# ZeldaM1/PnP-VCVE

Hardware: AMD Instinct MI355X
Metric: enhanced frames/sec (1280x720, 7-frame window) (higher is better)
Workload: dtype f32; 1 GPU; 1 x 7x3x720x1280 clip per GPU per step (BASELINE configs[2] shape), full BAE+CAA forward, config HR_davis_LR_128x128 generator, seeded random weights; side info per SURVEY 8(d): partition class ~ U{0,1,2} per 8x8 block (one-hot/255, none on the I frame), quarter-pel block MVs, IBBBP cadence; vsr_x4_heads=False, hip_graphs=False, deform=vos, parallelism=clip-sharded replicas x1

## Files before the change

### include/pnpvcve.h

```cpp
#ifndef PNPVCVE_H
#define PNPVCVE_H
#include <stddef.h>
#include <stdint.h>
#ifdef __cplusplus
extern "C" {
#endif

#define PNP_ERR_BAD_ARG 1001
#define PNP_ERR_UNSUPPORTED 1002
#define PNP_ERR_WORKSPACE 1003
#define PNP_ERR_SIZE_ASSERT 1004
#define PNP_ERR_SIZE_VALUE 1005

int pnp_abi_version(void);

typedef struct pnp_generator_cfg {
    int mid_channels;
    int num_blocks;
    int num_experts;
    int with_cat, use_base_qp, expert_softmax, with_bias, with_se;
    int one_layer, channel_first, align_key, vsr;
    int deform;
    int sparse_val;
    int num_group;
// ... 31 lines not shown
#define PNP_OPT_TILE_QUEUE 8
#define PNP_OPT_WINOGRAD 9
#define PNP_WINO_UNITS_MAX_TILES 128
#define PNP_OPT_COUNT 10
int pnp_generator_set_option(pnp_generator* g, int option, int value);
int pnp_generator_get_option(const pnp_generator* g, int option);

int pnp_generator_pack(const pnp_generator* g, const float* flat_dev, float* packed_dev, void* stream);

#define PNP_MAX_CONTEXTS 8
int64_t pnp_generator_workspace_bytes(const pnp_generator* g, int t, int h, int w);

int pnp_generator_set_max_resident(pnp_generator* g, int k);
int pnp_generator_get_max_resident(const pnp_generator* g);
int pnp_generator_min_resident(const pnp_generator* g, int t);

int pnp_generator_forward(const pnp_generator* g, const float* flat_dev, const float* packed_dev,
                          const float* lrs_dev, const float* mvs_dev, const float* par_dev,
                          const float* slices_host, const float* qps_host, const float* base_qps_host,
                          float* out_dev, void* workspace_dev, int64_t workspace_bytes,
                          int n, int t, int h, int w, void* stream);

#define PNP_PROF_CONV_BLOCK 0
#define PNP_PROF_CONV_INPUT 1
#define PNP_PROF_CONV_HEAD 2
#define PNP_PROF_WARP 3
#define PNP_PROF_DCN 4
int pnp_generator_profile(pnp_generator* g, int enable);
int pnp_generator_profile_read(pnp_generator* g, int kind, double* total_ms, int64_t* launches, double* work);

// ... 93 lines not shown
```

### include/pnpvcve_debug.h

```cpp
#ifndef PNPVCVE_DEBUG_H
#define PNPVCVE_DEBUG_H
#include "pnpvcve.h"
#ifdef __cplusplus
extern "C" {
#endif

#define PNP_CONV_AUTO 0
#define PNP_CONV_TILE 1
#define PNP_CONV_TILE_BIG 2

int pnp_conv3x3_f32_ex(int nsrc, const float* const* srcs_dev, const int* src_channels,
                       const float* const* packed_w_dev, const float* bias_dev, const float* gamma_dev,
                       const float* packed_w1x1_dev, const float* par_dev, const float* residual_dev,
                       int act, float* out_dev, int h, int w, int variant, const int* par_flags_dev,
                       void* trace_dev, void* stream);

int pnp_conv3x3_wino_f32_ex(const float* src_dev, const float* wino_w_dev, const float* bias_dev, const float* gamma_dev,
                            const float* wino_w1x1_dev, const float* par_dev, const int* par_flags_dev,
                            const float* residual_dev, int act, float* out_dev, int h, int w, void* trace_dev, void* stream);
int pnp_debug_wino_gate_word(const int* gate_word_dev);

int pnp_conv3x3_f16_ex(int nsrc, const float* const* srcs_dev, const int* src_channels,
                       const void* const* packed_w_f16_dev, const float* bias_dev, const float* gamma_dev,
                       const void* packed_w1x1_f16_dev, const float* par_dev, const float* residual_dev,
                       int act, float* out_dev, int h, int w, void* trace_dev, void* stream);

int pnp_dcn_trace_u64s(void);
int pnp_dcn_nhwc_f32_ex(const float* x_dev, const float* om_dev, const float* flow_x_dev, const float* flow_y_dev,
                        const float* w_packed_dev, const float* bias_dev, float* out_dev, int h, int w, void* trace_dev,
                        void* stream);

int pnp_conv3x3_f16_maps(int nsrc, const void* const* srcs_dev, const int* src_channels, int src_f16_mask,
                         const void* const* packed_w_f16_dev, const float* bias_dev, const float* gamma_dev,
                         const void* packed_w1x1_f16_dev, const float* par_dev, const int* par_flags_dev,
                         const float* residual_dev, int act, void* out_dev, int out_f16, void* out16_dev, int h, int w,
// ... 16 lines not shown
```

### pnp_vcve_amd/_native.py

```python
import ctypes
import os
from ctypes import POINTER, c_char_p, c_float, c_int, c_int64, c_void_p

_HERE = os.path.dirname(os.path.abspath(__file__))
LIB_PATH = os.path.join(_HERE, 'lib', 'libpnpvcve_hip.so')

PNP_ERR = {1001: 'bad argument', 1002: 'unsupported configuration', 1003: 'workspace too small or misaligned',
           1004: 'size assert', 1005: 'size value'}


class GeneratorCfg(ctypes.Structure):
    _fields_ = [(k, c_int) for k in (
        'mid_channels', 'num_blocks', 'num_experts', 'with_cat', 'use_base_qp', 'expert_softmax', 'with_bias',
        'with_se', 'one_layer', 'channel_first', 'align_key', 'vsr', 'deform', 'sparse_val', 'num_group', 'flow_inter',
        'blocktype')]


SIGNATURES = {
    'pnp_abi_version': (c_int, []),
    'pnp_generator_create': (c_int, [POINTER(GeneratorCfg), POINTER(c_void_p)]),
    'pnp_generator_destroy': (None, [c_void_p]),
    'pnp_generator_num_params': (c_int, [c_void_p]),
    'pnp_generator_param_name': (c_char_p, [c_void_p, c_int]),
    'pnp_generator_param_ndim': (c_int, [c_void_p, c_int]),
    'pnp_generator_param_dim': (c_int64, [c_void_p, c_int, c_int]),
    'pnp_generator_param_offset': (c_int64, [c_void_p, c_int]),
    'pnp_generator_flat_floats': (c_int64, [c_void_p]),
    'pnp_generator_packed_floats': (c_int64, [c_void_p]),
    'pnp_generator_pack': (c_int, [c_void_p, c_void_p, c_void_p, c_void_p]),
    'pnp_generator_workspace_bytes': (c_int64, [c_void_p, c_int, c_int, c_int]),
    'pnp_generator_set_max_resident': (c_int, [c_void_p, c_int]),
    'pnp_generator_get_max_resident': (c_int, [c_void_p]),
    'pnp_generator_min_resident': (c_int, [c_void_p, c_int]),
    'pnp_generator_forward': (c_int, [c_void_p, c_void_p, c_void_p, c_void_p, c_void_p, c_void_p,
                                      POINTER(c_float), POINTER(c_float), POINTER(c_float),
                                      c_void_p, c_void_p, c_int64, c_int, c_int, c_int, c_int, c_void_p]),
    'pnp_generator_set_precision': (c_int, [c_void_p, c_int]),
    'pnp_generator_get_precision': (c_int, [c_void_p]),
    'pnp_generator_set_option': (c_int, [c_void_p, c_int, c_int]),
    'pnp_generator_get_option': (c_int, [c_void_p, c_int]),
    'pnp_generator_profile': (c_int, [c_void_p, c_int]),
    'pnp_generator_profile_read': (c_int, [c_void_p, c_int, POINTER(ctypes.c_double), POINTER(c_int64),
                                           POINTER(ctypes.c_double)]),
    'pnp_flow_warp_nchw_f32': (c_int, [c_void_p, c_void_p, c_void_p, c_int, c_int, c_int, c_int, c_void_p]),
    'pnp_mv_warp_nhwc_f32': (c_int, [c_void_p, c_void_p, c_void_p, c_void_p, c_int, c_int, c_int, c_void_p]),
    'pnp_flow_warp_nchw_mode_f32': (c_int, [c_void_p, c_void_p, c_void_p, c_int, c_int, c_int, c_int, c_int, c_void_p]),
    'pnp_mv_warp_nhwc_mode_f32': (c_int, [c_void_p, c_void_p, c_void_p, c_void_p, c_int, c_int, c_int, c_int, c_void_p]),
# ... 46 lines not shown
    'pnp_conv3x3_f16x3_ex': (c_int, [c_int, POINTER(c_void_p), POINTER(c_int), POINTER(c_void_p), POINTER(c_void_p),
                                     c_void_p, c_void_p, c_void_p, c_void_p, c_void_p, c_void_p,
                                     c_int, c_void_p, c_int, c_int, c_int, c_void_p, c_void_p, c_void_p]),
    'pnp_conv3x3_f32_ex': (c_int, [c_int, POINTER(c_void_p), POINTER(c_int), POINTER(c_void_p), c_void_p, c_void_p,
                                   c_void_p, c_void_p, c_void_p, c_int, c_void_p, c_int, c_int, c_int, c_void_p,
                                   c_void_p, c_void_p]),
    'pnp_conv3x3_f16_ex': (c_int, [c_int, POINTER(c_void_p), POINTER(c_int), POINTER(c_void_p), c_void_p, c_void_p,
                                   c_void_p, c_void_p, c_void_p, c_int, c_void_p, c_int, c_int, c_void_p, c_void_p]),
}

DEBUG_SIGNATURES['pnp_dcn_nhwc_f32_ex'] = (c_int, [c_void_p, c_void_p, c_void_p, c_void_p, c_void_p, c_void_p, c_void_p, c_int,
                                                   c_int, c_void_p, c_void_p])

DEBUG_SIGNATURES['pnp_dcn_trace_u64s'] = (c_int, [])
DEBUG_SIGNATURES['pnp_debug_wino_gate_word'] = (c_int, [c_void_p])
DEBUG_SIGNATURES['pnp_conv3x3_wino_f32_ex'] = (c_int, [c_void_p] * 8 + [c_int, c_void_p, c_int, c_int, c_void_p, c_void_p])
DEBUG_SIGNATURES['pnp_conv3x3_f16_maps'] = (c_int, [c_int, POINTER(c_void_p), POINTER(c_int), c_int, POINTER(c_void_p), c_void_p,
                                                    c_void_p, c_void_p, c_void_p, c_void_p, c_void_p, c_int, c_void_p, c_int, c_void_p,
                                                    c_int, c_int, c_int, c_void_p, c_void_p])
DEBUG_SIGNATURES['pnp_mv_warp_nhwc_f16out'] = (c_int, [c_void_p, c_void_p, c_void_p, c_void_p, c_int, c_int, c_int, c_void_p])

(OPT_F16_MAPS, OPT_PAR_SKIP, OPT_CONV_LAST_VALU, OPT_PERSIST, OPT_SMALL_F16, OPT_SPARSE_EVAL, OPT_F16_MIRRORS, OPT_F16_CHAIN_MIRRORS,
 OPT_TILE_QUEUE, OPT_WINOGRAD) = range(10)
CONV_AUTO, CONV_TILE, CONV_TILE_BIG = range(3)
WINO_UNITS_MAX_TILES = 128


def wino_kernel_form(h, w, wopt):
    if wopt <= 0:
        return None
# ... 34 lines not shown
```

### pnp_vcve_amd/csrc/conv_mfma.h

```cpp
#pragma once
#include "common.h"

struct ConvArgs {
    const float* src[4];
    const float* wsrc[4];
    int src_c[4];
    int nsrc;
    const float* wpar;
    const float* wwino;
    const float* wwino_par;
    const float* wwino_src[4];
    const float* wwino_rgb;
    const int* par_any;
    int wino_units;
    const float* wvalu;
    const void* wsrc_h[4];
    const void* wpar_h;
    int wpar_h_scaled;
    int* tile_queue;
    int prec;
    int src_f16, out_f16;
    void* out16;
    int no_multi16;
    const float* par;
    const int* par_flags;
    long par_plane;
    const float* bias;
    const float* gamma;
// ... 93 lines not shown
```

### pnp_vcve_amd/csrc/conv_wino.hip

```cpp
#include "conv_mfma.h"
#include <cstring>
#include <type_traits>

namespace {

template <int N>
using I = std::integral_constant<int, N>;
typedef unsigned u32x4 __attribute__((ext_vector_type(4)));

constexpr int HP = 18, NPX = HP * HP;
constexpr int SLAB_B = NPX * 64;
constexpr int RING_B = 4 * 16384;
constexpr int PV_B = RING_B + 4 * SLAB_B;
constexpr int BG_B = PV_B + 256 * 48;
constexpr int DUMP_B = BG_B + 256;
constexpr int WINO_LDS = DUMP_B + 1024;
constexpr unsigned OOBW = 0xFFFFFFF0u;

__device__ __forceinline__ f32x4 mfma16(float a, float b, f32x4 c) { return __builtin_amdgcn_mfma_f32_16x16x4f32(a, b, c, 0, 0, 0); }
__device__ __forceinline__ __amdgpu_buffer_rsrc_t rsrc_of(const void* p, unsigned bytes) {
    return __builtin_amdgcn_make_buffer_rsrc(const_cast<void*>(p), 0, __builtin_amdgcn_readfirstlane((int)bytes), 0x00020000);
}
__device__ __forceinline__ f32x4 bload4(__amdgpu_buffer_rsrc_t r, unsigned voff, unsigned soff) {
    return __builtin_bit_cast(f32x4, __builtin_amdgcn_raw_buffer_load_b128(r, (int)voff, (int)soff, 0));
// ... 25 lines not shown
    long par_plane;
    const int* par_flags;
    const float *bias, *gamma, *residual;
    float* out;
    int H, W, act;
    unsigned long long* dbg;
    const float* srcs[3];
    unsigned u_off[3];
    const float* ubase;
    int nsrc;
    const float* rgb;
    const float* Urgb;
    const int* gate;
    int gate_mask, gate_want;
    int quad;
};

template <bool PAR, bool RES, bool MS, bool FO = false>
__device__ __forceinline__ void wino_tile_body(const WinoArgs& a) {
    static_assert(!MS || (!PAR && !RES), "the multi-source form is the input conv: no branches, no residual");
    static_assert(!FO || (!PAR && !MS), "fold-only is the plain structure");
    extern __shared__ __attribute__((aligned(16))) char smem[];
    const int t = threadIdx.x, lane = t & 63, wave = t >> 6;
    const int m = lane & 15, kq = lane >> 4;
    const int H = a.H, W = a.W;
    const int tiles_x = (W + 15) >> 4, ntiles = tiles_x * ((H + 15) >> 4);
    constexpr bool MSF = MS;
    constexpr bool SEAM = PAR;
    if (a.gate) {
        const int gv = __builtin_nontemporal_load(a.gate);
        if (((gv & a.gate_mask) != 0) != (a.gate_want != 0)) return;
    }

    int tile, tstep, tend, qtile = -1, qquad = 0;
    if ((gridDim.x & 7) == 0) {
        const int xcd = blockIdx.x & 7, slot = blockIdx.x >> 3;
        const int bq = ntiles >> 3, br = ntiles & 7;
        const int xbeg = xcd < br ? xcd * (bq + 1) : br * (bq + 1) + (xcd - br) * bq;
        tend = xbeg + bq + (xcd < br ? 1 : 0);
        tile = xbeg + slot;
        tstep = gridDim.x >> 3;
        const int nband = tend - xbeg, rounds = nband / tstep, left = nband - rounds * tstep;
        if (!MS && a.quad && rounds >= 1 && left > 0 && 4 * left <= tstep) {
            tend = xbeg + rounds * tstep;
            if (slot < 4 * left) {
                qtile = tend + (slot >> 2);
                qquad = slot & 3;
            }
        }
    } else {
        tile = blockIdx.x;
        tstep = gridDim.x;
        tend = ntiles;
    }
    if (tile >= tend) return;

    const unsigned map_bytes = (unsigned)H * (unsigned)W * 256u;
    __amdgpu_buffer_rsrc_t r_src = rsrc_of(reinterpret_cast<const char*>(MS ? a.srcs[0] : a.src) - ((long)W + 1) * 256, OOBW);
    const __amdgpu_buffer_rsrc_t r_u = rsrc_of(MS ? a.ubase : a.U, MS ? OOBW : 16u * 16384u);
    const __amdgpu_buffer_rsrc_t r_urgb = rsrc_of(MS ? a.Urgb : a.U, 4u * 4096u);
    const __amdgpu_buffer_rsrc_t r_rgb = rsrc_of(reinterpret_cast<const char*>(MS ? a.rgb : a.src) - ((long)W + 1) * 16, OOBW);
    const __amdgpu_buffer_rsrc_t r_up = rsrc_of((PAR || FO) ? a.Upar : a.U, 4u * 12288u);
    const __amdgpu_buffer_rsrc_t r_out = rsrc_of(a.out, map_bytes);
    const __amdgpu_buffer_rsrc_t r_res = rsrc_of(RES ? a.residual : a.src, RES ? map_bytes : 0u);
    const __amdgpu_buffer_rsrc_t r_par = rsrc_of(a.par, PAR ? (unsigned)(3 * a.par_plane * 4) : 0u);

    const unsigned t16 = (unsigned)t * 16u;
    const int ty = 4 * (wave >> 1) + (m >> 2), tx = 4 * (wave & 1) + (m & 3);
// ... 1279 lines not shown
    if (!a.wwino_rgb || a.prec != 0 || cfg == CONV_CFG_RGB || grid_y != 1 || a.out_mode != 0) return false;
    if (a.nsrc < 2 || a.nsrc > 4 || a.src_c[0] != 4 || a.src_f16 || a.out_f16 || a.out16) return false;
    if (a.wpar || a.residual || a.gamma) return false;
    for (int s = 1; s < a.nsrc; ++s)
        if (a.src_c[s] != 64 || !a.wwino_src[s]) return false;
    return (long)a.H * a.W * 256 < ((long)1 << 32) - 65536;
}

bool conv_wino_eligible(const ConvArgs& a, int cfg, int grid_y) {
    if (!a.wwino || a.prec != 0 || cfg == CONV_CFG_RGB || grid_y != 1 || a.out_mode != 0) return false;
    if (a.nsrc != 1 || a.src_c[0] != 64 || a.src_f16 || a.out_f16 || a.out16) return false;
    if (a.wpar && (!a.wwino_par || !a.par)) return false;
    return (long)a.H * a.W * 256 < ((long)1 << 32) - 65536;
}

int launch_conv3x3_wino(const ConvArgs& a, hipStream_t stream) {
    static PnpPerDevice once;
    int cus = 256;
    const hipError_t attr_err = once.run([](int dev, int& g) {
        hipError_t e = hipSuccess;
        const void* fo = reinterpret_cast<const void*>(conv3x3_wino_gated_kernel<false>);
        e = hipFuncSetAttribute(fo, hipFuncAttributeMaxDynamicSharedMemorySize, WINO_LDS);
        const void* fo_res = reinterpret_cast<const void*>(conv3x3_wino_gated_kernel<true>);
        if (e == hipSuccess) e = hipFuncSetAttribute(fo_res, hipFuncAttributeMaxDynamicSharedMemorySize, WINO_LDS);
        const void* fns[4] = {reinterpret_cast<const void*>(conv3x3_wino_kernel<false, false, false>),
                              reinterpret_cast<const void*>(conv3x3_wino_kernel<false, true, false>),
                              reinterpret_cast<const void*>(conv3x3_wino_kernel<true, false, false>),
                              reinterpret_cast<const void*>(conv3x3_wino_kernel<true, true, false>)};
        for (int i = 0; i < 4 && e == hipSuccess; ++i) e = hipFuncSetAttribute(fns[i], hipFuncAttributeMaxDynamicSharedMemorySize, WINO_LDS);
        g = 256;
        (void)hipDeviceGetAttribute(&g, hipDeviceAttributeMultiprocessorCount, dev);
// ... 5 lines not shown
    w.src = a.src[0];
    w.U = a.wwino;
    w.Upar = a.wpar ? a.wwino_par : nullptr;
    w.par = a.par;
    w.par_plane = a.par_plane;
    w.par_flags = a.par_flags;
    w.bias = a.bias;
    w.gamma = a.gamma;
    w.residual = a.residual;
    w.out = a.out;
    w.H = a.H;
    w.W = a.W;
    w.act = a.act;
    w.dbg = a.dbg;
    w.quad = 1;
    const int ntiles = ((a.W + 15) / 16) * ((a.H + 15) / 16);
    if (a.wino_units && a.wwino) {
        const dim3 gq(4 * ntiles), bq(256);
        if (a.wpar && a.par_any) {
            w.gate = a.par_any;
            if (a.residual) hipLaunchKernelGGL((conv3x3_wino_quad_gated_kernel<true>), gq, bq, 0, stream, w);
            else hipLaunchKernelGGL((conv3x3_wino_quad_gated_kernel<false>), gq, bq, 0, stream, w);
        } else if (a.wpar && a.residual) hipLaunchKernelGGL((conv3x3_wino_quad_kernel<true, true>), gq, bq, 0, stream, w);
        else if (a.wpar) hipLaunchKernelGGL((conv3x3_wino_quad_kernel<true, false>), gq, bq, 0, stream, w);
        else if (a.residual) hipLaunchKernelGGL((conv3x3_wino_quad_kernel<false, true>), gq, bq, 0, stream, w);
        else hipLaunchKernelGGL((conv3x3_wino_quad_kernel<false, false>), gq, bq, 0, stream, w);
        return (int)hipGetLastError();
    }
    if (a.residual && a.act != 0) return PNP_ERR_UNSUPPORTED;
    int grid = ntiles < cus ? ntiles : cus;
    if (grid >= 8) grid -= grid % 8;
// ... 27 lines not shown
```

### pnp_vcve_amd/csrc/generator.hip

```cpp
#include <string>
#include <vector>
#include <cstring>
#include <cstdlib>

#include "../../include/pnpvcve.h"
#include "../../include/pnpvcve_debug.h"
#include "abi_shared.h"
#include "conv_mfma.h"
#include "prep.h"
#include "warp.h"
#include "dcn.h"

namespace {

struct ParamInfo {
    std::string name;
    std::vector<int64_t> shape;
    int64_t offset = 0, numel = 0;
};

struct BlockPk {
    int64_t conv1_img = -1;
    int64_t conv1_bias = -1;
    int64_t conv2_img = -1;
// ... 23 lines not shown

struct pnp_generator {
    pnp_generator_cfg cfg;
    int prec = PNP_PREC_F32;
    int opt[PNP_OPT_COUNT] = {1, 1, 1, 1, 1, 1, 1, 0, 1, 1};
    int max_resident = 0;
    mutable bool prof_on = false;
    mutable std::vector<hipEvent_t> prof_pool;
    mutable size_t prof_used = 0;
    mutable std::vector<ProfRec> prof_recs;
    mutable hipEvent_t prof_last = nullptr;
    mutable hipStream_t prof_last_stream = nullptr;
    mutable std::vector<hipStream_t> side_streams;
    mutable std::vector<hipEvent_t> join_events;
    mutable hipEvent_t fork_event = nullptr;
    std::vector<ParamInfo> params;
    int64_t flat_floats = 0, packed_floats = 0;
    int ndyn = 0;
    int64_t dyn_w = 0, dyn_b = 0;
    BranchPk br[2];
    int64_t hr_img = -1, hr_bias = -1, last_img = -1, last_bias = -1;
    int64_t hr_wino = -1;
    int64_t ones2 = -1;
    int64_t last_valu = -1;
    int64_t up_img[2] = {-1, -1}, up_bias[2] = {-1, -1};
    int64_t f_dcn_b = -1, f_off0_b = -1, f_off2_b = -1;
    int64_t dcn_img = -1, off0_flow_img = -1, off0_feat_img = -1, off2_img = -1, off2_bias = -1;
    int64_t p_w1 = -1, p_b1 = -1, p_w2 = -1, p_b2 = -1, p_v1 = -1, p_v2 = -1;
    std::vector<WeightImage> images;
    int64_t f_last_w = -1, f_last_b = -1, f_up_b[2] = {-1, -1};
// ... 329 lines not shown
                *R = r;
                *L = l;
                return true;
            }
    return false;
}

int plan_min_resident(int t, int with_cat) {
    int R, L, k = 1;
    while (!plan_pick(t, with_cat, k, &R, &L)) ++k;
    return k;
}

bool bounded_mode(const pnp_generator* g, int t) { return g->max_resident > 0 && g->max_resident < t; }

struct Step {
    int sweep, frame, key_frame;
    int out, key, nb, own;
};

bool make_schedule(const pnp_generator* g, int t, const std::vector<char>& key, std::vector<Step>& steps, int* recomputed) {
    const int cat = g->cfg.with_cat;
    steps.clear();
    *recomputed = 0;
    auto nk = [&](int i) { int k = i + 1; while (!key[k]) ++k; return k; };
    auto pk = [&](int i) { int k = i - 1; while (!key[k]) --k; return k; };
    if (!bounded_mode(g, t)) {
        for (int i = t - 1; i >= 0; --i)
            steps.push_back({0, i, i < t - 1 ? nk(i) : -1, i, i < t - 1 ? nk(i) : -1, (cat && i < t - 1) ? i + 1 : -1, -1});
        for (int i = 0; i < t; ++i)
// ... 132 lines not shown
    const int rc = build_layout(g);
    if (rc != PNP_OK) {
        delete g;
        return rc;
    }
    *out = g;
    return PNP_OK;
}

void pnp_generator_destroy(pnp_generator* g) {
    if (!g) return;
    for (hipEvent_t e : g->prof_pool) (void)hipEventDestroy(e);
    for (hipEvent_t e : g->join_events) (void)hipEventDestroy(e);
    for (hipStream_t s : g->side_streams) (void)hipStreamDestroy(s);
    if (g->fork_event) (void)hipEventDestroy(g->fork_event);
    delete g;
}

int pnp_generator_num_params(const pnp_generator* g) { return (int)g->params.size(); }
const char* pnp_generator_param_name(const pnp_generator* g, int i) { return g->params[i].name.c_str(); }
int pnp_generator_param_ndim(const pnp_generator* g, int i) { return (int)g->params[i].shape.size(); }
int64_t pnp_generator_param_dim(const pnp_generator* g, int i, int d) { return g->params[i].shape[d]; }
int64_t pnp_generator_param_offset(const pnp_generator* g, int i) { return g->params[i].offset; }
int64_t pnp_generator_flat_floats(const pnp_generator* g) { return g->flat_floats; }
int64_t pnp_generator_packed_floats(const pnp_generator* g) {
    const int halves = g->prec == PNP_PREC_F16 ? 1 : (g->prec == PNP_PREC_F16X3 ? 2 : 0);
    return g->packed_floats + halves * (g->packed_floats / 2);
}

int pnp_generator_set_precision(pnp_generator* g, int precision) {
// ... 77 lines not shown
    return (int)hipGetLastError();
}

int64_t pnp_generator_workspace_bytes(const pnp_generator* g, int t, int h, int w) {
    int R, L;
    if (bounded_mode(g, t) && !plan_pick(t, g->cfg.with_cat, g->max_resident, &R, &L)) return -1;
    return carve(g, nullptr, t, h, w).bytes;
}

int pnp_generator_set_max_resident(pnp_generator* g, int k) {
    if (!g || k < 0) return PNP_ERR_BAD_ARG;
    g->max_resident = k;
    return PNP_OK;
}
int pnp_generator_get_max_resident(const pnp_generator* g) { return g ? g->max_resident : -1; }
int pnp_generator_min_resident(const pnp_generator* g, int t) {
    if (!g || t < 1) return -1;
    return plan_min_resident(t, g->cfg.with_cat);
}

}

namespace {

int forward_sample(const pnp_generator* g, const float* flat, const float* packed, const float* lr_b, const float* mv_b,
                   const float* par_b, const float* sl, const float* qp, const float* bq, float* out_b,
                   const Workspace& W, int t, int h, int w, hipStream_t st) {
    const auto& c = g->cfg;
    const int64_t hw = (int64_t)h * w, fm = hw * 64;
    const int E = c.num_experts;
    const int cfg_lr = conv_pick_cfg(h, w);
    const int os = c.vsr ? 4 : 1;
    int rc;

    const int64_t n_mix = (int64_t)t * g->ndyn * IMG_WIDE;
    auto twin = [&](const float* p) -> const void* {
        if (g->prec == PNP_PREC_F32 || !p) return nullptr;
        const int64_t halfs = g->prec == PNP_PREC_F16X3 ? 2 : 1;
        if (p >= packed && p < packed + g->packed_floats)
            return reinterpret_cast<const uint16_t*>(packed + g->packed_floats) + halfs * (p - packed);
        if (p >= W.mixw && p < W.mixw + n_mix) return reinterpret_cast<const uint16_t*>(W.mixh) + halfs * (p - W.mixw);
        return nullptr;
    };
    const bool f16_maps = g->prec == PNP_PREC_F16 && g->opt[PNP_OPT_F16_MAPS];
    const bool par_skip = g->opt[PNP_OPT_PAR_SKIP] != 0;
    const int wopt = g->prec == PNP_PREC_F32 ? g->opt[PNP_OPT_WINOGRAD] : 0;
    auto ntiles16 = [](int hh, int ww) { return (int64_t)((hh + 15) / 16) * ((ww + 15) / 16); };
    const bool wino_on = wopt != 0;
    auto wino_units = [&](int hh, int ww) { return wopt == 1 && ntiles16(hh, ww) <= PNP_WINO_UNITS_MAX_TILES; };
    const bool mirrors = f16_maps && g->opt[PNP_OPT_F16_MIRRORS] && c.deform == 0 && W.x16 != nullptr;
    const bool chain16 = mirrors && g->opt[PNP_OPT_F16_CHAIN_MIRRORS];
    auto conv = [&](const ConvCall& q) -> int {
        ConvArgs a;
        memset(&a, 0, sizeof(a));
        a.nsrc = q.nsrc;
        a.prec = g->prec;
        for (int s = 0; s < q.nsrc; ++s) {
            a.src[s] = q.src[s];
            a.src_c[s] = q.sc[s];
            a.wsrc[s] = q.w[s];
            a.wsrc_h[s] = twin(q.w[s]);
        }
        a.wpar = q.wpar_;
        a.wwino = q.wino_;
        a.wwino_par = q.wino_par_;
        if (q.nsrc >= 2 && q.sc[0] == 4 && q.wsrc_wino_[0]) {
// ... 30 lines not shown
        if (mirrors) {
            for (int s = 0; s < q.nsrc; ++s)
                if (q.src16_[s]) {
                    a.src[s] = reinterpret_cast<const float*>(q.src16_[s]);
                    a.src_f16 |= 1 << s;
                }
            a.out16 = q.out16_;
        }
        double kreal = 0;
        for (int s = 0; s < q.nsrc; ++s) kreal += 9.0 * (q.sc[s] == 64 ? 64 : 3);
        if (q.wpar_) kreal += 3 * 64;
        const double nreal = (q.mode_ == 2 || q.mode_ == 3) ? 3 : 64;
        const int kind = (q.mode_ != 0) ? PNP_PROF_CONV_HEAD
                                        : (q.nsrc > 1 || q.sc[0] != 64) ? PNP_PROF_CONV_INPUT : PNP_PROF_CONV_BLOCK;
        ProfScope ps(g, st, kind, 2.0 * kreal * nreal * (double)q.H * q.W * q.gy_);
        return launch_conv3x3(a, q.cfg_, q.gy_, st);
    };

    auto align = [&](const float* feat, const float* fxp, const float* fyp) -> int {
        int r;
        if (c.deform == 0 || c.deform == 1) {
            ProfScope ps(g, st, PNP_PROF_WARP, (mirrors ? 392.0 : 520.0) * (double)hw);
            r = launch_mv_warp_nhwc(feat, fxp, fyp, c.deform == 0 ? W.kw : W.tmp0, h, w, 64, st, mirrors, c.flow_inter == 1);
            if (r || c.deform == 0) return r;
        }
        r = launch_pack_flow4(fxp, fyp, W.flow4, h, w, st);
        g->prof_last = nullptr;
        if (r) return r;
        r = conv(ConvCall(h, w, cfg_lr).source(W.flow4, 4, packed + g->off0_flow_img)
                     .source(c.deform == 1 ? W.tmp0 : feat, 64, packed + g->off0_feat_img)
// ... 199 lines not shown
                if (rc) return rc;
                if (c.with_cat && c.align_key && sp.key_frame == (sp.sweep == 0 ? i + 1 : i - 1)) {
                    in.source(W.kw, 64, packed + B.in_wide01, wi(B.in_wide01_wino)).mirror16(kw16);
                } else {
                    in.source(W.kw, 64, packed + B.in_wide[0], wi(B.in_wide_wino[0])).mirror16(kw16);
                    if (c.with_cat) in.source(slot_of(sp.nb), 64, packed + B.in_wide[1], wi(B.in_wide_wino[1])).mirror16(s16of(sp.nb));
                }
            }
            if (sp.sweep == 1)
                in.source(slot_of(sp.own), 64, packed + B.in_wide[B.n_wide - 1], wi(B.in_wide_wino[B.n_wide - 1])).mirror16(s16of(sp.own));
            if (sparse_per_frame) {
                rc = launch_par_sparse(par_in + (int64_t)i * 3 * hw, W.parbin, 1, h, w, st);
                g->prof_last = nullptr;
                if (rc) return rc;
            }
            rc = run_branch(sp.sweep, i, sp.out, in);
            if (rc) return rc;
            if (sp.sweep == 0) continue;

            const float* feat = slot_of(sp.out);
            const float* lr_i = lr_b + (int64_t)i * 3 * hw;
            float* out_i = out_b + (int64_t)i * 3 * hw * os * os;
            const int o16 = f16_maps ? 1 : 0, s16 = f16_maps ? 2 : 0;
            if (!c.vsr) {
                rc = conv(ConvCall(h, w, cfg_lr).source(feat, 64, packed + g->hr_img).mirror16(s16of(sp.out)).bias(flat + g->hr_bias)
                              .wino(wino_on ? packed + g->hr_wino : nullptr).units(wino_units(h, w)).act(2).to(W.tmp1).f16_map(o16));
                if (!rc)
                    rc = conv(ConvCall(h, w, CONV_CFG_RGB).source(W.tmp1, 64, packed + g->last_img).bias(packed + g->last_bias)
                                  .mode(2).rgb(lr_i, hw, packed + g->last_valu).to(out_i).f16_map(s16));
                if (rc) return rc;
            } else {
                rc = conv(ConvCall(h, w, cfg_lr).source(feat, 64, packed + g->up_img[0]).bias(packed + g->up_bias[0], 64)
                              .act(2).mode(1, 4, IMG_WIDE).to(W.u1).f16_map(o16));
                if (!rc)
                    rc = conv(ConvCall(2 * h, 2 * w, conv_pick_cfg(2 * h, 2 * w)).source(W.u1, 64, packed + g->up_img[1])
                                  .bias(packed + g->up_bias[1], 64).act(2).mode(1, 4, IMG_WIDE).to(W.u2).f16_map(o16 | s16));
                if (!rc)
                    rc = conv(ConvCall(4 * h, 4 * w, conv_pick_cfg(4 * h, 4 * w)).source(W.u2, 64, packed + g->hr_img)
                                  .bias(flat + g->hr_bias).wino(wino_on ? packed + g->hr_wino : nullptr).units(wino_units(4 * h, 4 * w)).act(2).to(W.u3)
                                  .f16_map(o16 | s16));
                if (!rc)
// ... 38 lines not shown
            if (err != hipSuccess) return (int)err;
            err = hipEventCreateWithFlags(&e, hipEventDisableTiming);
            if (err != hipSuccess) return (int)err;
            g->side_streams.push_back(s);
            g->join_events.push_back(e);
        }
        if (!g->fork_event) {
            const hipError_t err = hipEventCreateWithFlags(&g->fork_event, hipEventDisableTiming);
            if (err != hipSuccess) return (int)err;
        }
        hipError_t err = hipEventRecord(g->fork_event, st);
        for (int k = 0; k < nctx && err == hipSuccess; ++k) err = hipStreamWaitEvent(g->side_streams[k], g->fork_event, 0);
        if (err != hipSuccess) return (int)err;
    }
    int rc = PNP_OK;
    for (int b = 0; b < n && rc == PNP_OK; ++b) {
        const int k = b % nctx;
        const Workspace W = carve(g, (char*)workspace + (int64_t)k * ctx_bytes, t, h, w);
        rc = forward_sample(g, flat, packed, lrs + (int64_t)b * t * 3 * hw, mvs + (int64_t)b * t * 4 * hw,
                            par + (int64_t)b * t * 3 * hw, slices + (int64_t)b * t, qps + (int64_t)b * t,
                            base_qps + (int64_t)b * t, out + (int64_t)b * t * 3 * hw * os * os, W, t, h, w,
                            nctx > 1 ? g->side_streams[k] : st);
    }
    if (nctx > 1) {
        for (int k = 0; k < nctx; ++k) {
            hipError_t err = hipEventRecord(g->join_events[k], g->side_streams[k]);
            if (err == hipSuccess) err = hipStreamWaitEvent(st, g->join_events[k], 0);
            if (err != hipSuccess && rc == PNP_OK) rc = (int)err;
        }
    }
    return rc;
}

int pnp_generator_profile(pnp_generator* g, int enable) {
    if (!g) return PNP_ERR_BAD_ARG;
    g->prof_on = enable != 0;
    g->prof_used = 0;
// ... 28 lines not shown
```

### pnp_vcve_amd/csrc/ops_abi.hip

```cpp
#include <cstring>

#include "../../include/pnpvcve.h"
#include "../../include/pnpvcve_debug.h"
#include "abi_shared.h"
#include "conv_mfma.h"
#include "warp.h"
#include "dcn.h"

namespace {

ConvArgs op_conv_args(int nsrc, const float* const* srcs, const int* src_channels, const float* bias, const float* gamma, const float* par,
                      const int* par_flags, const float* residual, int act, float* out, int h, int w, void* trace) {
    ConvArgs a;
    memset(&a, 0, sizeof(a));
    a.nsrc = nsrc;
    for (int s = 0; s < nsrc; ++s) {
        a.src[s] = srcs[s];
        a.src_c[s] = src_channels[s];
    }
    a.par = par;
    a.par_flags = par_flags;
    a.par_plane = (long)h * w;
    a.bias = bias;
    a.gamma = gamma;
// ... 135 lines not shown
    return launch_pack_weights(plain_pack(w, 64, 1, PACK_1X1, 0, 2, 64, dst), 1, (hipStream_t)st);
}

int64_t pnp_wino_image_floats(void) { return PNP_WINO_IMG_FLOATS; }
int64_t pnp_wino_par_image_floats(void) { return PNP_WINO_PAR_FLOATS; }

int64_t pnp_wino_rgb_image_floats(void) { return PNP_WINO_RGB_FLOATS; }

int pnp_wino_rgb_image_from_packed_f32(const float* packed_rgb_chunk, float* dst, void* st) {
    return launch_wino_rgb_image(packed_rgb_chunk, dst, (hipStream_t)st);
}

static int wino_ms_op(int nsrc, const float* const* srcs, const float* const* wino_w, const float* bias, int act, float* out,
                      int h, int w, int units, void* st);

int pnp_conv3x3_wino_ms_f32(int nsrc, const float* const* srcs, const float* const* wino_w, const float* bias, int act, float* out,
                            int h, int w, void* st) {
    return wino_ms_op(nsrc, srcs, wino_w, bias, act, out, h, w, 0, st);
}

int pnp_conv3x3_wino_ms_units_f32(int nsrc, const float* const* srcs, const float* const* wino_w, const float* bias, int act,
                                  float* out, int h, int w, void* st) {
    return wino_ms_op(nsrc, srcs, wino_w, bias, act, out, h, w, 1, st);
}

static int wino_ms_op(int nsrc, const float* const* srcs, const float* const* wino_w, const float* bias, int act, float* out,
                      int h, int w, int units, void* st) {
    if (nsrc < 2 || nsrc > 4 || !srcs || !wino_w || !out || act < 0 || act > 2) return PNP_ERR_BAD_ARG;
    if (!op_map_fits(h, w)) return PNP_ERR_UNSUPPORTED;
    static const int channels[4] = {4, 64, 64, 64};
    ConvArgs a = op_conv_args(nsrc, srcs, channels, bias, nullptr, nullptr, nullptr, nullptr, act, out, h, w, nullptr);
    for (int s = 0; s < nsrc; ++s) {
        if (!srcs[s] || !wino_w[s]) return PNP_ERR_BAD_ARG;
        a.wwino_src[s] = wino_w[s];
    }
    a.wwino_rgb = wino_w[0];
    a.wino_units = units;
    if (!conv_wino_ms_eligible(a, CONV_CFG_BIG, 1)) return PNP_ERR_UNSUPPORTED;
    return launch_conv3x3_wino(a, (hipStream_t)st);
}

int pnp_wino_image_from_packed_f32(const float* packed_w, const float* gamma, float* dst, void* st) {
    return launch_wino_images(&packed_w, &dst, 1, gamma, (hipStream_t)st);
}

int pnp_wino_par_image_from_packed_f32(const float* packed_w1x1, float* dst, void* st) {
    return launch_wino_par_image(packed_w1x1, dst, (hipStream_t)st);
}

int pnp_conv3x3_wino_f32(const float* src, const float* wino_w, const float* bias, const float* gamma, const float* wino_w1x1,
                         const float* par, const int* par_flags, const float* residual, int act, float* out, int h, int w,
                         void* st) {
// ... 15 lines not shown

int pnp_conv3x3_wino_f32_ex(const float* src, const float* wino_w, const float* bias, const float* gamma, const float* wino_w1x1,
                            const float* par, const int* par_flags, const float* residual, int act, float* out, int h, int w,
                            void* trace, void* st) {
    if (!src || !wino_w || !out || act < 0 || act > 2 || (wino_w1x1 && !par)) return PNP_ERR_BAD_ARG;
    if (!op_map_fits(h, w)) return PNP_ERR_UNSUPPORTED;
    const int channels = 64;
    const bool units = trace == (void*)&pnp_conv3x3_wino_units_f32;
    ConvArgs a = op_conv_args(1, &src, &channels, bias, gamma, wino_w1x1 ? par : nullptr, wino_w1x1 ? par_flags : nullptr, residual, act,
                              out, h, w, units ? nullptr : trace);
    a.wwino = wino_w;
    a.wwino_par = wino_w1x1;
    a.wpar = wino_w1x1;
    a.par_any = (wino_w1x1 && par_flags) ? g_debug_wino_gate_word : nullptr;
    a.wino_units = units ? 1 : 0;
    if (!conv_wino_eligible(a, CONV_CFG_BIG, 1)) return PNP_ERR_UNSUPPORTED;
    return launch_conv3x3_wino(a, (hipStream_t)st);
}

int pnp_conv3x3_f32(int nsrc, const float* const* srcs, const int* src_channels, const float* const* packed_w,
                    const float* bias, const float* gamma, const float* packed_w1x1, const float* par,
                    const float* residual, int act, float* out, int h, int w, void* st) {
    return pnp_conv3x3_f32_ex(nsrc, srcs, src_channels, packed_w, bias, gamma, packed_w1x1, par, residual, act, out, h, w,
                              PNP_CONV_AUTO, nullptr, nullptr, st);
}

int pnp_conv3x3_f32_ex(int nsrc, const float* const* srcs, const int* src_channels, const float* const* packed_w,
                       const float* bias, const float* gamma, const float* packed_w1x1, const float* par,
                       const float* residual, int act, float* out, int h, int w, int variant, const int* par_flags,
                       void* trace, void* st) {
// ... 145 lines not shown
```

### pnp_vcve_amd/generator.py

```python
import ctypes
import math

import torch
import torch.nn as nn

from . import _native
from .registry import BACKBONES

_DEFORM = {'vos': 0, 'basic': 1, 'fvc': 2}
_FLOW_INTER = {'bilinear': 0, 'nearest': 1}
_BLOCKTYPES = {'drt': 0, 'drt_woqp': 1}


def _kaiming_normal_fan_in(t, scale):
    nn.init.kaiming_normal_(t, a=0, mode='fan_in', nonlinearity='relu')
    t.data.mul_(scale)


@BACKBONES.register_module()
class IconVSR_restore_wo_refill_mv_ipb_fast_domain_dynamic_with_par(nn.Module):
    def __init__(self, mid_channels=64, num_blocks=30, num_experts=10, num_group=1, expert_softmax=False,
                 use_base_qp=False, with_bias=False, with_se=False, with_par=False, init_weight=False,
                 one_layer=False, small_sft=False, blocktype='default', channel_first=False, drconv=False,
                 sparse_val=False, vsr=False, align_key=False,
# ... 94 lines not shown

    @property
    def max_resident_features(self):
        k = int(_native.lib().pnp_generator_get_max_resident(self._handle))
        return None if k == 0 else k

    @max_resident_features.setter
    def max_resident_features(self, value):
        if value is not None and (isinstance(value, bool) or not isinstance(value, int) or value < 1):
            raise ValueError(f'max_resident_features must be None or a positive int, got {value!r}')
        _native.check(_native.lib().pnp_generator_set_max_resident(self._handle, 0 if value is None else int(value)),
                      'pnp_generator_set_max_resident')
        self._workspace = {}
        self._graphs = {}

    def min_resident_features(self, t):
        if int(t) < 1:
            raise ValueError(f't must be >= 1, got {t!r}')
        return int(_native.lib().pnp_generator_min_resident(self._handle, int(t)))

    def _check_resident(self, t):
        k = self.max_resident_features
        if k is not None and k < t and k < self.min_resident_features(t):
            raise ValueError(f'max_resident_features={k} is below the minimum {self.min_resident_features(t)} for a clip of {t} frames')

    def _register(self, dotted, param):
        mod = self
        parts = dotted.split('.')
        for p in parts[:-1]:
            if p not in mod._modules:
# ... 203 lines not shown
```

### pnp_vcve_amd/ops.py

```python
import ctypes

import torch

from . import _native


def _stream():
    return ctypes.c_void_p(torch.cuda.current_stream().cuda_stream)


def _ptr(t):
    return ctypes.c_void_p(t.data_ptr()) if t is not None else ctypes.c_void_p(0)


def _on_device_of_first_tensor(fn):
    import functools

    @functools.wraps(fn)
    def wrapped(*args, **kwargs):
        first = next((a for a in args if isinstance(a, torch.Tensor)), None)
        if first is None:
            first = next((a[0] for a in args if isinstance(a, (list, tuple)) and a and isinstance(a[0], torch.Tensor)), None)
        if first is not None and first.is_cuda:
            with torch.cuda.device(first.device):
# ... 287 lines not shown
    _native.check(_native.lib().pnp_wino_par_image_from_packed_f32(_ptr(packed_w1x1), _ptr(out), _stream()),
                  'pnp_wino_par_image_from_packed_f32')
    return out


@_on_device_of_first_tensor
def wino_rgb_image(packed_rgb):
    packed_rgb = _chk(packed_rgb, 'packed_rgb')
    out = torch.empty(int(_native.lib().pnp_wino_rgb_image_floats()), device=packed_rgb.device, dtype=torch.float32)
    _native.check(_native.lib().pnp_wino_rgb_image_from_packed_f32(_ptr(packed_rgb), _ptr(out), _stream()),
                  'pnp_wino_rgb_image_from_packed_f32')
    return out


@_on_device_of_first_tensor
def conv3x3_wino_ms(srcs, wino_ws, bias=None, act=0, units=False):
    srcs = [_chk(x, 'src') for x in srcs]
    wino_ws = [_chk(x, 'wino_w') for x in wino_ws]
    h, w = srcs[0].shape[:2]
    n = len(srcs)
    if n != len(wino_ws) or srcs[0].shape[2] != 4 or any(x.shape != (h, w, 64) for x in srcs[1:]):
        raise ValueError('srcs must be [(h,w,4), (h,w,64) ...] with one Winograd image each')
    out = torch.empty((h, w, 64), device=srcs[0].device, dtype=torch.float32)
    sp = (ctypes.c_void_p * n)(*[x.data_ptr() for x in srcs])
    wp = (ctypes.c_void_p * n)(*[x.data_ptr() for x in wino_ws])
    fn = _native.lib().pnp_conv3x3_wino_ms_units_f32 if units else _native.lib().pnp_conv3x3_wino_ms_f32
    _native.check(fn(n, sp, wp, _ptr(_chk(bias, 'bias')) if bias is not None else None, int(act), _ptr(out), h, w, _stream()),
                  'pnp_conv3x3_wino_ms_f32')
    return out


@_on_device_of_first_tensor
def conv3x3_wino(x, wino_w, bias=None, gamma=None, wino_w1x1=None, par=None, par_flags=None, residual=None, act=0, trace=None, units=False):
    x = _chk(x, 'x')
    h, w, c = x.shape
    if c != 64:
        raise ValueError('x must be (h, w, 64)')
    tag = getattr(wino_w, '_pnp_gamma', 'untagged')
    if not isinstance(tag, str) and ((tag is None) != (gamma is None) or (gamma is not None and not torch.equal(tag, gamma))):
        raise ValueError('conv3x3_wino: `gamma` scales only the bias -- the conv term carries the gain wino_image() folded into wino_w; '
                         'pass the SAME gamma tensor to both (or none to both)')
    out = torch.empty_like(x)
    opt = lambda t, n: _ptr(_chk(t, n)) if t is not None else None
    if par_flags is not None and (par_flags.dtype != torch.int32 or not par_flags.is_cuda):
        raise ValueError('par_flags must be a CUDA int32 tensor')
    args = (_ptr(x), _ptr(_chk(wino_w, 'wino_w')), opt(bias, 'bias'), opt(gamma, 'gamma'), opt(wino_w1x1, 'wino_w1x1'), opt(par, 'par'),
            ctypes.c_void_p(par_flags.data_ptr()) if par_flags is not None else None, opt(residual, 'residual'), int(act), _ptr(out), h, w)
    if units:
        _native.check(_native.lib().pnp_conv3x3_wino_units_f32(*args, _stream()), 'pnp_conv3x3_wino_units_f32')
    elif trace is None:
        _native.check(_native.lib().pnp_conv3x3_wino_f32(*args, _stream()), 'pnp_conv3x3_wino_f32')
    else:
        _native.check(_native.lib().pnp_conv3x3_wino_f32_ex(*args, ctypes.c_void_p(trace.data_ptr()), _stream()), 'pnp_conv3x3_wino_f32_ex')
    return out


@_on_device_of_first_tensor
# ... 126 lines not shown
```

Before: 88.86 frames/s.

## Split Winograd conv chains into row bands overlapped across two streams

New measurement: 92.21 frames/s (median of 6 runs). 1.04x the previous value.

```diff
diff --git a/include/pnpvcve.h b/include/pnpvcve.h
--- a/include/pnpvcve.h
+++ b/include/pnpvcve.h
@@ -69,6 +69,9 @@
 int pnp_generator_set_max_resident(pnp_generator* g, int k);
 int pnp_generator_get_max_resident(const pnp_generator* g);
 int pnp_generator_min_resident(const pnp_generator* g, int t);
+
+int pnp_generator_set_band_split(pnp_generator* g, int on);
+int pnp_generator_get_band_split(const pnp_generator* g);
 
 int pnp_generator_forward(const pnp_generator* g, const float* flat_dev, const float* packed_dev,
                           const float* lrs_dev, const float* mvs_dev, const float* par_dev,
diff --git a/include/pnpvcve_debug.h b/include/pnpvcve_debug.h
--- a/include/pnpvcve_debug.h
+++ b/include/pnpvcve_debug.h
@@ -19,6 +19,10 @@
                             const float* wino_w1x1_dev, const float* par_dev, const int* par_flags_dev,
                             const float* residual_dev, int act, float* out_dev, int h, int w, void* trace_dev, void* stream);
 int pnp_debug_wino_gate_word(const int* gate_word_dev);
+
+int pnp_debug_wino_tile_rows(int row0, int nrows);
+
+int pnp_band_plan(int rows, int nconv, int a0, int* bounds);
 
 int pnp_conv3x3_f16_ex(int nsrc, const float* const* srcs_dev, const int* src_channels,
                        const void* const* packed_w_f16_dev, const float* bias_dev, const float* gamma_dev,
diff --git a/pnp_vcve_amd/_native.py b/pnp_vcve_amd/_native.py
--- a/pnp_vcve_amd/_native.py
+++ b/pnp_vcve_amd/_native.py
@@ -31,6 +31,8 @@
     'pnp_generator_workspace_bytes': (c_int64, [c_void_p, c_int, c_int, c_int]),
     'pnp_generator_set_max_resident': (c_int, [c_void_p, c_int]),
     'pnp_generator_get_max_resident': (c_int, [c_void_p]),
+    'pnp_generator_set_band_split': (c_int, [c_void_p, c_int]),
+    'pnp_generator_get_band_split': (c_int, [c_void_p]),
     'pnp_generator_min_resident': (c_int, [c_void_p, c_int]),
     'pnp_generator_forward': (c_int, [c_void_p, c_void_p, c_void_p, c_void_p, c_void_p, c_void_p,
                                       POINTER(c_float), POINTER(c_float), POINTER(c_float),
@@ -107,6 +109,8 @@
 
 DEBUG_SIGNATURES['pnp_dcn_trace_u64s'] = (c_int, [])
 DEBUG_SIGNATURES['pnp_debug_wino_gate_word'] = (c_int, [c_void_p])
+DEBUG_SIGNATURES['pnp_debug_wino_tile_rows'] = (c_int, [c_int, c_int])
+DEBUG_SIGNATURES['pnp_band_plan'] = (c_int, [c_int, c_int, c_int, POINTER(c_int)])
 DEBUG_SIGNATURES['pnp_conv3x3_wino_f32_ex'] = (c_int, [c_void_p] * 8 + [c_int, c_void_p, c_int, c_int, c_void_p, c_void_p])
 DEBUG_SIGNATURES['pnp_conv3x3_f16_maps'] = (c_int, [c_int, POINTER(c_void_p), POINTER(c_int), c_int, POINTER(c_void_p), c_void_p,
                                                     c_void_p, c_void_p, c_void_p, c_void_p, c_void_p, c_int, c_void_p, c_int, c_void_p,
diff --git a/pnp_vcve_amd/csrc/conv_mfma.h b/pnp_vcve_amd/csrc/conv_mfma.h
--- a/pnp_vcve_amd/csrc/conv_mfma.h
+++ b/pnp_vcve_amd/csrc/conv_mfma.h
@@ -1,5 +1,11 @@
 #pragma once
 #include "common.h"
+
+struct ConvBandSplit {
+    hipStream_t side;
+    hipEvent_t ready;
+    int row;
+};
 
 struct ConvArgs {
     const float* src[4];
@@ -12,6 +18,8 @@
     const float* wwino_src[4];
     const float* wwino_rgb;
     const int* par_any;
+    int tile_row0, tile_rows;
+    const ConvBandSplit* band;
     int wino_units;
     const float* wvalu;
     const void* wsrc_h[4];
diff --git a/pnp_vcve_amd/csrc/conv_wino.hip b/pnp_vcve_amd/csrc/conv_wino.hip
--- a/pnp_vcve_amd/csrc/conv_wino.hip
+++ b/pnp_vcve_amd/csrc/conv_wino.hip
@@ -63,6 +63,7 @@
     const int* gate;
     int gate_mask, gate_want;
     int quad;
+    int tile0, tcount;
 };
 
 template <bool PAR, bool RES, bool MS, bool FO = false>
@@ -73,7 +74,7 @@
     const int t = threadIdx.x, lane = t & 63, wave = t >> 6;
     const int m = lane & 15, kq = lane >> 4;
     const int H = a.H, W = a.W;
-    const int tiles_x = (W + 15) >> 4, ntiles = tiles_x * ((H + 15) >> 4);
+    const int tiles_x = (W + 15) >> 4;
     constexpr bool MSF = MS;
     constexpr bool SEAM = PAR;
     if (a.gate) {
@@ -84,8 +85,8 @@
     int tile, tstep, tend, qtile = -1, qquad = 0;
     if ((gridDim.x & 7) == 0) {
         const int xcd = blockIdx.x & 7, slot = blockIdx.x >> 3;
-        const int bq = ntiles >> 3, br = ntiles & 7;
-        const int xbeg = xcd < br ? xcd * (bq + 1) : br * (bq + 1) + (xcd - br) * bq;
+        const int bq = a.tcount >> 3, br = a.tcount & 7;
+        const int xbeg = a.tile0 + (xcd < br ? xcd * (bq + 1) : br * (bq + 1) + (xcd - br) * bq);
         tend = xbeg + bq + (xcd < br ? 1 : 0);
         tile = xbeg + slot;
         tstep = gridDim.x >> 3;
@@ -98,9 +99,9 @@
             }
         }
     } else {
-        tile = blockIdx.x;
+        tile = a.tile0 + blockIdx.x;
         tstep = gridDim.x;
-        tend = ntiles;
+        tend = a.tile0 + a.tcount;
     }
     if (tile >= tend) return;
 
@@ -1410,7 +1411,26 @@
     return (long)a.H * a.W * 256 < ((long)1 << 32) - 65536;
 }
 
+static int launch_wino_rows(const ConvArgs& a, int row0, int nrows, hipStream_t stream);
+
 int launch_conv3x3_wino(const ConvArgs& a, hipStream_t stream) {
+    const int rows = (a.H + 15) / 16;
+    if (!a.band) {
+        if (a.tile_rows == 0) return launch_wino_rows(a, 0, rows, stream);
+        if (a.wino_units || a.tile_row0 < 0 || a.tile_rows < 0 || a.tile_row0 + a.tile_rows > rows) return PNP_ERR_BAD_ARG;
+        return launch_wino_rows(a, a.tile_row0, a.tile_rows, stream);
+    }
+    const ConvBandSplit& b = *a.band;
+    if (a.wino_units || a.tile_rows != 0 || b.row < 1 || b.row >= rows || !b.ready) return PNP_ERR_BAD_ARG;
+    hipError_t e = hipEventRecord(b.ready, stream);
+    if (e == hipSuccess) e = hipStreamWaitEvent(b.side, b.ready, 0);
+    if (e != hipSuccess) return (int)e;
+    int rc = launch_wino_rows(a, 0, b.row, stream);
+    if (rc) return rc;
+    return launch_wino_rows(a, b.row, rows - b.row, b.side);
+}
+
+static int launch_wino_rows(const ConvArgs& a, int row0, int nrows, hipStream_t stream) {
     static PnpPerDevice once;
     int cus = 256;
     const hipError_t attr_err = once.run([](int dev, int& g) {
@@ -1446,7 +1466,10 @@
     w.act = a.act;
     w.dbg = a.dbg;
     w.quad = 1;
-    const int ntiles = ((a.W + 15) / 16) * ((a.H + 15) / 16);
+    const int tiles_x = (a.W + 15) / 16;
+    const int ntiles = tiles_x * nrows;
+    w.tile0 = tiles_x * row0;
+    w.tcount = ntiles;
     if (a.wino_units && a.wwino) {
         const dim3 gq(4 * ntiles), bq(256);
         if (a.wpar && a.par_any) {
diff --git a/pnp_vcve_amd/csrc/generator.hip b/pnp_vcve_amd/csrc/generator.hip
--- a/pnp_vcve_amd/csrc/generator.hip
+++ b/pnp_vcve_amd/csrc/generator.hip
@@ -1,3 +1,4 @@
+#include <deque>
 #include <string>
 #include <vector>
 #include <cstring>
@@ -61,6 +62,10 @@
     mutable std::vector<hipStream_t> side_streams;
     mutable std::vector<hipEvent_t> join_events;
     mutable hipEvent_t fork_event = nullptr;
+    int band_split = 1;
+    mutable hipStream_t band_stream = nullptr;
+    mutable std::vector<hipEvent_t> band_events;
+    mutable std::deque<ConvBandSplit> band_recs;
     std::vector<ParamInfo> params;
     int64_t flat_floats = 0, packed_floats = 0;
     int ndyn = 0;
@@ -420,6 +425,14 @@
 
 bool bounded_mode(const pnp_generator* g, int t) { return g->max_resident > 0 && g->max_resident < t; }
 
+bool band_plan(int rows, int nconv, int a0, int* first) {
+    if (rows < 1 || nconv < 1 || a0 < 0) return false;
+    const int a = a0 > 0 ? a0 : (rows + nconv - 1) / 2;
+    if (a - (nconv - 1) < 1 || a > rows - 1) return false;
+    *first = a;
+    return true;
+}
+
 struct Step {
     int sweep, frame, key_frame;
     int out, key, nb, own;
@@ -582,6 +595,8 @@
     for (hipEvent_t e : g->join_events) (void)hipEventDestroy(e);
     for (hipStream_t s : g->side_streams) (void)hipStreamDestroy(s);
     if (g->fork_event) (void)hipEventDestroy(g->fork_event);
+    for (hipEvent_t e : g->band_events) (void)hipEventDestroy(e);
+    if (g->band_stream) (void)hipStreamDestroy(g->band_stream);
     delete g;
 }
 
@@ -689,6 +704,18 @@
     return PNP_OK;
 }
 int pnp_generator_get_max_resident(const pnp_generator* g) { return g ? g->max_resident : -1; }
+int pnp_generator_set_band_split(pnp_generator* g, int on) {
+    if (!g || on < 0) return PNP_ERR_BAD_ARG;
+    g->band_split = on;
+    return PNP_OK;
+}
+int pnp_generator_get_band_split(const pnp_generator* g) { return g ? g->band_split : -1; }
+int pnp_band_plan(int rows, int nconv, int a0, int* bounds) {
+    int first;
+    if (!bounds || nconv > 4096 || !band_plan(rows, nconv, a0, &first)) return 0;
+    for (int n = 0; n < nconv; ++n) bounds[n] = first - n;
+    return 1;
+}
 int pnp_generator_min_resident(const pnp_generator* g, int t) {
     if (!g || t < 1) return -1;
     return plan_min_resident(t, g->cfg.with_cat);
@@ -700,7 +727,7 @@
 
 int forward_sample(const pnp_generator* g, const float* flat, const float* packed, const float* lr_b, const float* mv_b,
                    const float* par_b, const float* sl, const float* qp, const float* bq, float* out_b,
-                   const Workspace& W, int t, int h, int w, hipStream_t st) {
+                   const Workspace& W, int t, int h, int w, hipStream_t st, bool alone) {
     const auto& c = g->cfg;
     const int64_t hw = (int64_t)h * w, fm = hw * 64;
     const int E = c.num_experts;
@@ -725,6 +752,45 @@
     auto wino_units = [&](int hh, int ww) { return wopt == 1 && ntiles16(hh, ww) <= PNP_WINO_UNITS_MAX_TILES; };
     const bool mirrors = f16_maps && g->opt[PNP_OPT_F16_MIRRORS] && c.deform == 0 && W.x16 != nullptr;
     const bool chain16 = mirrors && g->opt[PNP_OPT_F16_CHAIN_MIRRORS];
+    const bool band_mode = alone && g->band_split != 0 && wopt != 0 && !wino_units(h, w);
+    struct {
+        bool open = false, forked = false;
+        int left = 0, n = 0, row = 0;
+    } chain;
+    auto chain_open = [&](int nconv) -> int {
+        if (!band_mode) return PNP_OK;
+        int first;
+        const int rows = (h + 15) / 16, a0 = g->band_split >= 2 ? g->band_split : 0;
+        if (!band_plan(rows, nconv, a0, &first) && !band_plan(rows, nconv - 1, a0, &first)) return PNP_OK;
+        if (!g->band_stream) {
+            const hipError_t e = hipStreamCreateWithFlags(&g->band_stream, hipStreamNonBlocking);
+            if (e != hipSuccess) return (int)e;
+        }
+        while ((int)g->band_events.size() < nconv + 1) {
+            hipEvent_t e;
+            const hipError_t err = hipEventCreateWithFlags(&e, hipEventDisableTiming);
+            if (err != hipSuccess) return (int)err;
+            g->band_events.push_back(e);
+        }
+        chain.open = true;
+        chain.forked = false;
+        chain.left = nconv;
+        chain.n = 0;
+        return PNP_OK;
+    };
+    auto chain_close = [&]() -> int {
+        const bool join = chain.open && chain.forked;
+        chain.open = chain.forked = false;
+        if (!join) return PNP_OK;
+        hipError_t e = hipEventRecord(g->band_events.back(), g->band_stream);
+        if (e == hipSuccess) e = hipStreamWaitEvent(st, g->band_events.back(), 0);
+        g->prof_last = nullptr;
+        return (int)e;
+    };
+    struct ChainGuard {
+        decltype(chain_close)& close;
+        ~ChainGuard() { (void)close(); }
+    } chain_guard{chain_close};
     auto conv = [&](const ConvCall& q) -> int {
         ConvArgs a;
         memset(&a, 0, sizeof(a));
@@ -785,6 +851,23 @@
         const int kind = (q.mode_ != 0) ? PNP_PROF_CONV_HEAD
                                         : (q.nsrc > 1 || q.sc[0] != 64) ? PNP_PROF_CONV_INPUT : PNP_PROF_CONV_BLOCK;
         ProfScope ps(g, st, kind, 2.0 * kreal * nreal * (double)q.H * q.W * q.gy_);
+        if (chain.open) {
+            const bool tiles = !a.wino_units && q.H == h && q.W == w && (conv_wino_eligible(a, q.cfg_, q.gy_) || conv_wino_ms_eligible(a, q.cfg_, q.gy_));
+            if (!tiles && chain.n > 0) return PNP_ERR_UNSUPPORTED;
+            if (tiles && chain.n == 0 && !band_plan((h + 15) / 16, chain.left, g->band_split >= 2 ? g->band_split : 0, &chain.row))
+                chain.open = false;
+            --chain.left;
+            if (tiles && chain.open) {
+                g->band_recs.emplace_back();
+                ConvBandSplit& band = g->band_recs.back();
+                memset(&band, 0, sizeof(band));
+                band.side = g->band_stream;
+                band.ready = g->band_events[chain.n++];
+                band.row = chain.row--;
+                a.band = &band;
+                chain.forked = true;
+            }
+        }
         return launch_conv3x3(a, q.cfg_, q.gy_, st);
     };
 
@@ -1014,7 +1097,11 @@
                 g->prof_last = nullptr;
                 if (rc) return rc;
             }
+            const bool hr_in_chain = sp.sweep == 1 && !c.vsr;
+            rc = chain_open(1 + 2 * c.num_blocks + (hr_in_chain ? 1 : 0));
+            if (rc) return rc;
             rc = run_branch(sp.sweep, i, sp.out, in);
+            if (!rc && !hr_in_chain) rc = chain_close();
             if (rc) return rc;
             if (sp.sweep == 0) continue;
 
@@ -1025,6 +1112,7 @@
             if (!c.vsr) {
                 rc = conv(ConvCall(h, w, cfg_lr).source(feat, 64, packed + g->hr_img).mirror16(s16of(sp.out)).bias(flat + g->hr_bias)
                               .wino(wino_on ? packed + g->hr_wino : nullptr).units(wino_units(h, w)).act(2).to(W.tmp1).f16_map(o16));
+                if (!rc) rc = chain_close();
                 if (!rc)
                     rc = conv(ConvCall(h, w, CONV_CFG_RGB).source(W.tmp1, 64, packed + g->last_img).bias(packed + g->last_bias)
                                   .mode(2).rgb(lr_i, hw, packed + g->last_valu).to(out_i).f16_map(s16));
@@ -1093,13 +1181,14 @@
         if (err != hipSuccess) return (int)err;
     }
     int rc = PNP_OK;
+    g->band_recs.clear();
     for (int b = 0; b < n && rc == PNP_OK; ++b) {
         const int k = b % nctx;
         const Workspace W = carve(g, (char*)workspace + (int64_t)k * ctx_bytes, t, h, w);
         rc = forward_sample(g, flat, packed, lrs + (int64_t)b * t * 3 * hw, mvs + (int64_t)b * t * 4 * hw,
                             par + (int64_t)b * t * 3 * hw, slices + (int64_t)b * t, qps + (int64_t)b * t,
                             base_qps + (int64_t)b * t, out + (int64_t)b * t * 3 * hw * os * os, W, t, h, w,
-                            nctx > 1 ? g->side_streams[k] : st);
+                            nctx > 1 ? g->side_streams[k] : st, nctx == 1);
     }
     if (nctx > 1) {
         for (int k = 0; k < nctx; ++k) {
diff --git a/pnp_vcve_amd/csrc/ops_abi.hip b/pnp_vcve_amd/csrc/ops_abi.hip
--- a/pnp_vcve_amd/csrc/ops_abi.hip
+++ b/pnp_vcve_amd/csrc/ops_abi.hip
@@ -173,6 +173,14 @@
 static int wino_ms_op(int nsrc, const float* const* srcs, const float* const* wino_w, const float* bias, int act, float* out,
                       int h, int w, int units, void* st);
 
+static int g_debug_wino_row0 = 0, g_debug_wino_rows = 0;
+int pnp_debug_wino_tile_rows(int row0, int nrows) {
+    if (row0 < 0 || nrows < 0) return PNP_ERR_BAD_ARG;
+    g_debug_wino_row0 = row0;
+    g_debug_wino_rows = nrows;
+    return 0;
+}
+
 int pnp_conv3x3_wino_ms_f32(int nsrc, const float* const* srcs, const float* const* wino_w, const float* bias, int act, float* out,
                             int h, int w, void* st) {
     return wino_ms_op(nsrc, srcs, wino_w, bias, act, out, h, w, 0, st);
@@ -195,6 +203,10 @@
     }
     a.wwino_rgb = wino_w[0];
     a.wino_units = units;
+    if (!units) {
+        a.tile_row0 = g_debug_wino_row0;
+        a.tile_rows = g_debug_wino_rows;
+    }
     if (!conv_wino_ms_eligible(a, CONV_CFG_BIG, 1)) return PNP_ERR_UNSUPPORTED;
     return launch_conv3x3_wino(a, (hipStream_t)st);
 }
@@ -240,6 +252,10 @@
     a.wpar = wino_w1x1;
     a.par_any = (wino_w1x1 && par_flags) ? g_debug_wino_gate_word : nullptr;
     a.wino_units = units ? 1 : 0;
+    if (!units) {
+        a.tile_row0 = g_debug_wino_row0;
+        a.tile_rows = g_debug_wino_rows;
+    }
     if (!conv_wino_eligible(a, CONV_CFG_BIG, 1)) return PNP_ERR_UNSUPPORTED;
     return launch_conv3x3_wino(a, (hipStream_t)st);
 }
diff --git a/pnp_vcve_amd/generator.py b/pnp_vcve_amd/generator.py
--- a/pnp_vcve_amd/generator.py
+++ b/pnp_vcve_amd/generator.py
@@ -132,6 +132,19 @@
         self._workspace = {}
         self._graphs = {}
 
+    @property
+    def band_split(self):
+        return int(_native.lib().pnp_generator_get_band_split(self._handle))
+
+    @band_split.setter
+    def band_split(self, value):
+        if isinstance(value, bool):
+            value = int(value)
+        if not isinstance(value, int) or value < 0:
+            raise ValueError(f'band_split must be an int >= 0, got {value!r}')
+        _native.check(_native.lib().pnp_generator_set_band_split(self._handle, value), 'pnp_generator_set_band_split')
+        self._graphs = {}
+
     def min_resident_features(self, t):
         if int(t) < 1:
             raise ValueError(f't must be >= 1, got {t!r}')
diff --git a/pnp_vcve_amd/ops.py b/pnp_vcve_amd/ops.py
--- a/pnp_vcve_amd/ops.py
+++ b/pnp_vcve_amd/ops.py
@@ -1,3 +1,4 @@
+import contextlib
 import ctypes
 
 import torch
@@ -325,14 +326,17 @@
 
 
 @_on_device_of_first_tensor
-def conv3x3_wino_ms(srcs, wino_ws, bias=None, act=0, units=False):
+def conv3x3_wino_ms(srcs, wino_ws, bias=None, act=0, units=False, out=None):
     srcs = [_chk(x, 'src') for x in srcs]
     wino_ws = [_chk(x, 'wino_w') for x in wino_ws]
     h, w = srcs[0].shape[:2]
     n = len(srcs)
     if n != len(wino_ws) or srcs[0].shape[2] != 4 or any(x.shape != (h, w, 64) for x in srcs[1:]):
         raise ValueError('srcs must be [(h,w,4), (h,w,64) ...] with one Winograd image each')
-    out = torch.empty((h, w, 64), device=srcs[0].device, dtype=torch.float32)
+    if out is None:
+        out = torch.empty((h, w, 64), device=srcs[0].device, dtype=torch.float32)
+    elif _chk(out, 'out').shape != (h, w, 64) or not out.is_contiguous():
+        raise ValueError('out must be a contiguous (h, w, 64) tensor')
     sp = (ctypes.c_void_p * n)(*[x.data_ptr() for x in srcs])
     wp = (ctypes.c_void_p * n)(*[x.data_ptr() for x in wino_ws])
     fn = _native.lib().pnp_conv3x3_wino_ms_units_f32 if units else _native.lib().pnp_conv3x3_wino_ms_f32
@@ -341,8 +345,18 @@
     return out
 
 
-@_on_device_of_first_tensor
-def conv3x3_wino(x, wino_w, bias=None, gamma=None, wino_w1x1=None, par=None, par_flags=None, residual=None, act=0, trace=None, units=False):
+@contextlib.contextmanager
+def wino_tile_rows(row0, nrows):
+    _native.check(_native.lib().pnp_debug_wino_tile_rows(int(row0), int(nrows)), 'pnp_debug_wino_tile_rows')
+    try:
+        yield
+    finally:
+        _native.lib().pnp_debug_wino_tile_rows(0, 0)
+
+
+@_on_device_of_first_tensor
+def conv3x3_wino(x, wino_w, bias=None, gamma=None, wino_w1x1=None, par=None, par_flags=None, residual=None, act=0, trace=None, units=False,
+                 out=None):
     x = _chk(x, 'x')
     h, w, c = x.shape
     if c != 64:
@@ -351,7 +365,10 @@
     if not isinstance(tag, str) and ((tag is None) != (gamma is None) or (gamma is not None and not torch.equal(tag, gamma))):
         raise ValueError('conv3x3_wino: `gamma` scales only the bias -- the conv term carries the gain wino_image() folded into wino_w; '
                          'pass the SAME gamma tensor to both (or none to both)')
-    out = torch.empty_like(x)
+    if out is None:
+        out = torch.empty_like(x)
+    elif _chk(out, 'out').shape != x.shape or not out.is_contiguous():
+        raise ValueError('out must be a contiguous tensor of the shape of x')
     opt = lambda t, n: _ptr(_chk(t, n)) if t is not None else None
     if par_flags is not None and (par_flags.dtype != torch.int32 or not par_flags.is_cuda):
         raise ValueError('par_flags must be a CUDA int32 tensor')
```
